# OpenRL-Lab/openrl

Measured on NVIDIA H100. Metric: env-steps/sec (collect+update), CartPole-v1 PPO, higher is better.
Workload: dtype f32 (nets, losses, Adam; the three 64x64 GEMM groups of the update run as split-fp16 wgmma MMAs with fp32 accumulation = fp32-class accuracy, the mode the 1e-4 parity tests run in), f64 (CartPole state)

## Files before the change

### openrl_b200/csrc/orl_fwd_tc.cu

```cuda
#include <algorithm>
#include <cstdlib>
#include <map>
#include <mutex>

#include "orl_envstep.cuh"
#include "orl_tc16.cuh"

namespace {
using namespace orl;
using namespace orl::tc;

constexpr int F_M = 128, F_NT = 256, FCW = 32;
constexpr uint32_t FPANEL = F_M * 16, FPANEL_W = H * 16;
constexpr int S_LD = 68;
constexpr uint32_t FOFF_R1H = 0, FOFF_R1L = 8 * FPANEL, FOFF_WH = 16 * FPANEL, FOFF_WL = FOFF_WH + 8 * FPANEL_W, FOFF_S = FOFF_WL + 8 * FPANEL_W,
                   FOFF_SMALL = FOFF_S + F_M * S_LD * 4;
constexpr uint32_t F_SMALL_FLOATS = 8 * H + H + H + MAX_OUT * H + MAX_OUT;
constexpr uint32_t F_XCH_FLOATS = 2 * F_M * 2 + 2 * F_M * 8 + F_M * 8;
constexpr uint32_t F_SMEM = FOFF_SMALL + 4 * (F_SMALL_FLOATS + F_XCH_FLOATS);

#define F_FOR_OUT(j) _Pragma("unroll") for (int j = 0; j < NOUT; ++j) if (NOUT != 8 || j < n)
#define F_ROWGROUP_SYNC()                                                      \
    do {                                                                       \
        switch (warp & 3) {                                                    \
// ... 76 lines not shown
    for (int i = 0; i < FCW; ++i) { n1[i] = f_act<ACT>(n1[i], activation_id); s += n1[i]; sq = fmaf(n1[i], n1[i], sq); }
    {
        *reinterpret_cast<float2*>(c.xs + (half * F_M + row) * 2) = make_float2(s, sq);
        F_ROWGROUP_SYNC();
        const float2 o = *reinterpret_cast<const float2*>(c.xs + ((half ^ 1) * F_M + row) * 2);
        s += o.x; sq += o.y;
    }
    const float mu1 = s * (1.f / H);
    const float rstd1 = 1.0f / sqrtf(fmaxf(sq * (1.f / H) - mu1 * mu1, 0.f) + LN_EPS);
#pragma unroll
    for (int i = 0; i < FCW; ++i) n1[i] = (n1[i] - mu1) * rstd1;
#pragma unroll
    for (int q8 = 0; q8 < FCW; q8 += 8) {
        const uint32_t off = (uint32_t)((cb + q8) >> 3) * FPANEL + row * 16;
        split_store8(c.R1h + off, c.R1l + off, n1 + q8, 1.0f);
    }
    fence_proxy_async();
    __syncthreads();
    {
        const uint64_t dK_A = desc_const(FPANEL, 128), dK_W = desc_const(FPANEL_W, 128);
        float z[32];
#pragma unroll
        for (int i = 0; i < 32; ++i) z[i] = 0.f;
        wgmma_fence();
#pragma unroll
        for (int pass = 0; pass < 3; ++pass) {
            const uint32_t aa = (pass == 0 ? c.aR1l : c.aR1h) + half * 64 * 16, bb = pass == 1 ? c.aWl : c.aWh;
#pragma unroll
            for (int kk = 0; kk < 4; ++kk)
                wgmma_f16_n64<0, 0>(z, desc_at(dK_A, aa + 2 * kk * FPANEL), desc_at(dK_W, bb + 2 * kk * FPANEL_W), (pass | kk) > 0);
        }
        wgmma_commit();
        overlap();
        wgmma_wait0();
        frag_store<64>(z, c.S + half * 64 * S_LD, S_LD);
    }
    __syncthreads();
    float n3[FCW];
#pragma unroll
    for (int q4 = 0; q4 < FCW; q4 += 4) {
        const float4 v = *reinterpret_cast<const float4*>(c.S + row * S_LD + cb + q4);
        n3[q4] = v.x; n3[q4 + 1] = v.y; n3[q4 + 2] = v.z; n3[q4 + 3] = v.w;
    }
    float s3 = 0.f, q3 = 0.f;
#pragma unroll
    for (int i = 0; i < FCW; ++i) { n3[i] += c.b3f[cb + i]; s3 += n3[i]; q3 = fmaf(n3[i], n3[i], q3); }
    {
        __syncwarp();
        *reinterpret_cast<float2*>(c.xs + (half * F_M + row) * 2) = make_float2(s3, q3);
        F_ROWGROUP_SYNC();
        const float2 o = *reinterpret_cast<const float2*>(c.xs + ((half ^ 1) * F_M + row) * 2);
        s3 += o.x; q3 += o.y;
    }
    const float mu3 = s3 * (1.f / H);
    const float rstd3 = 1.0f / sqrtf(fmaxf(q3 * (1.f / H) - mu3 * mu3, 0.f) + LN_EPS);
#pragma unroll
    for (int j = 0; j < MAX_OUT; ++j) out[j] = 0.f;
#pragma unroll
    for (int q4 = 0; q4 < FCW; q4 += 4) {
#pragma unroll
        for (int i = 0; i < 4; ++i) n3[q4 + i] = (n3[q4 + i] - mu3) * rstd3;
        F_FOR_OUT(j) {
            const float4 wv = *reinterpret_cast<const float4*>(c.whf + j * H + cb + q4);
            out[j] = fmaf(n3[q4], wv.x, fmaf(n3[q4 + 1], wv.y, fmaf(n3[q4 + 2], wv.z, fmaf(n3[q4 + 3], wv.w, out[j]))));
        }
    }
    {
// ... 229 lines not shown
            *reinterpret_cast<float2*>(xs + (qd * F_M + row) * 2) = make_float2(sm, sq);
            Q_ROWGROUP_SYNC();
            {
                sm = 0.f; sq = 0.f;
#pragma unroll
                for (int p = 0; p < 4; ++p) { const float2 o = *reinterpret_cast<const float2*>(xs + (p * F_M + row) * 2); sm += o.x; sq += o.y; }
            }
            const float mu1 = sm * (1.f / H);
            const float rstd1 = 1.0f / sqrtf(fmaxf(sq * (1.f / H) - mu1 * mu1, 0.f) + LN_EPS);
#pragma unroll
            for (int i = 0; i < QCW; ++i) n1[i] = (n1[i] - mu1) * rstd1;
#pragma unroll
            for (int q8 = 0; q8 < QCW; q8 += 8) {
                const uint32_t off = (uint32_t)((cb + q8) >> 3) * FPANEL + row * 16;
                split_store8(c.R1h + off, c.R1l + off, n1 + q8, 1.0f);
            }
            fence_proxy_async();
            Q_FWD_SYNC();
            {
                const uint64_t dK_A = desc_const(FPANEL, 128), dK_W = desc_const(FPANEL_W, 128);
                const int mb = qd & 1, nb = qd >> 1;
                float z[16];
#pragma unroll
                for (int i = 0; i < 16; ++i) z[i] = 0.f;
                wgmma_fence();
#pragma unroll
                for (int pass = 0; pass < 3; ++pass) {
                    const uint32_t aa = (pass == 0 ? c.aR1l : c.aR1h) + mb * 64 * 16, bb = (pass == 1 ? c.aWl : c.aWh) + nb * 32 * 16;
#pragma unroll
                    for (int kk = 0; kk < 4; ++kk)
                        wgmma_f16_n32<0, 0>(z, desc_at(dK_A, aa + 2 * kk * FPANEL), desc_at(dK_W, bb + 2 * kk * FPANEL_W), (pass | kk) > 0);
                }
                wgmma_commit();
                wgmma_wait0();
                frag_store<32>(z, c.S + mb * 64 * S_LD + 32 * nb, S_LD);
            }
            Q_FWD_SYNC();
            float n3[QCW];
#pragma unroll
            for (int q4 = 0; q4 < QCW; q4 += 4) {
                const float4 v = *reinterpret_cast<const float4*>(c.S + row * S_LD + cb + q4);
                n3[q4] = v.x; n3[q4 + 1] = v.y; n3[q4 + 2] = v.z; n3[q4 + 3] = v.w;
            }
            float s3 = 0.f, q3 = 0.f;
#pragma unroll
            for (int i = 0; i < QCW; ++i) { n3[i] += c.b3f[cb + i]; s3 += n3[i]; q3 = fmaf(n3[i], n3[i], q3); }
            __syncwarp();
            *reinterpret_cast<float2*>(xs + (qd * F_M + row) * 2) = make_float2(s3, q3);
            Q_ROWGROUP_SYNC();
            {
                s3 = 0.f; q3 = 0.f;
#pragma unroll
                for (int p = 0; p < 4; ++p) { const float2 o = *reinterpret_cast<const float2*>(xs + (p * F_M + row) * 2); s3 += o.x; q3 += o.y; }
            }
            const float mu3 = s3 * (1.f / H);
            const float rstd3 = 1.0f / sqrtf(fmaxf(q3 * (1.f / H) - mu3 * mu3, 0.f) + LN_EPS);
            float out[MAX_OUT];
#pragma unroll
            for (int j = 0; j < MAX_OUT; ++j) out[j] = 0.f;
#pragma unroll
            for (int q4 = 0; q4 < QCW; q4 += 4) {
#pragma unroll
                for (int i = 0; i < 4; ++i) n3[q4 + i] = (n3[q4 + i] - mu3) * rstd3;
                F_FOR_OUT(j) {
                    const float4 wv = *reinterpret_cast<const float4*>(c.whf + j * H + cb + q4);
                    out[j] = fmaf(n3[q4], wv.x, fmaf(n3[q4 + 1], wv.y, fmaf(n3[q4 + 2], wv.z, fmaf(n3[q4 + 3], wv.w, out[j]))));
                }
// ... 118 lines not shown
```

### openrl_b200/csrc/orl_ppo_tc.cu

```cuda
#include <cuda.h>

#include <algorithm>
#include <cstdlib>
#include <cstring>
#include <map>
#include <mutex>

#include "orl_mlp.cuh"
#include "orl_tc16.cuh"

namespace orl {
int ppo_stride_host(int obs_dim, int critic_obs_dim, int n_actions);
}

namespace {
using namespace orl;
using namespace orl::tc;

constexpr int T_M = 128, T_NT = 256;
constexpr int CW = 32;
constexpr uint32_t PANEL = T_M * 16;
constexpr uint32_t PANEL_W = H * 16;
constexpr int R1_PANELS = 10, R2_PANELS = 9;
constexpr int P_CST = 8, P_X = 9, P_U = 8;
constexpr int N_LOSS_TC = 8;
constexpr int S_LD = 68, GA_LD = 84, GB_LD = 20;
constexpr uint32_t OFF_R1H = 0, OFF_R1L = OFF_R1H + R1_PANELS * PANEL, OFF_R2H = OFF_R1L + R1_PANELS * PANEL,
                   OFF_R2L = OFF_R2H + R2_PANELS * PANEL, OFF_WH = OFF_R2L + R2_PANELS * PANEL, OFF_WL = OFF_WH + 8 * PANEL_W,
                   OFF_S = OFF_WL + 8 * PANEL_W, OFF_STAGE = OFF_S + T_M * S_LD * 4;
static_assert((T_M * GA_LD + 64 * GB_LD) * 4 <= OFF_WH, "the Ga / Gb staging fits in R1 + R2");
static_assert(OFF_STAGE % 128 == 0, "TMA destination alignment");
static_assert(OFF_R2L + 16 * PANEL <= OFF_STAGE + 4096, "the 16-panel A descriptors stay inside the allocation");
constexpr int N_SCAL = 4;

struct TcMaps {
    CUtensorMap obs_p, obs_c, actions, old_logp, adv, value_preds, returns, active;
};

struct AdvNormTc { float m0, s0, m1, s1; bool two; };

#define FOR_OUT(j) _Pragma("unroll") for (int j = 0; j < NOUT; ++j) if (NOUT != 8 || j < n)
#define ROWGROUP_SYNC()                                                        \
    do {                                                                       \
        switch (warp & 3) {                                                    \
            case 0: asm volatile("bar.sync 1, 64;" ::: "memory"); break;       \
            case 1: asm volatile("bar.sync 2, 64;" ::: "memory"); break;       \
            case 2: asm volatile("bar.sync 3, 64;" ::: "memory"); break;       \
            default: asm volatile("bar.sync 4, 64;" ::: "memory"); break;      \
        }                                                                      \
    } while (0)

__host__ __device__ inline uint32_t tc_stage_bytes(int d) { return (uint32_t)((T_M * d * 4 + 127) & ~127) + N_SCAL * T_M * 4; }
__host__ __device__ inline uint32_t tc_small_off(int d) { return OFF_STAGE + tc_stage_bytes(d); }
constexpr uint32_t SMALL_FLOATS = 8 * H + H + H + MAX_OUT * H + 2 * MAX_OUT;
constexpr uint32_t XCH_FLOATS = 2 * T_M * 2 + 2 * T_M * 8;
__host__ __device__ inline uint32_t tc_smem_bytes(int d) { return tc_small_off(d) + 4 * (SMALL_FLOATS + XCH_FLOATS) + 8; }

template <int ACT>
__device__ __forceinline__ float act_fwd_t(float z, int activation_id) { return ACT == 1 ? fmaxf(z, 0.f) : act_fwd(z, activation_id); }
template <int ACT>
__device__ __forceinline__ float act_bwd_t(float a, bool pos, int activation_id) { return ACT == 1 ? (pos ? 1.f : 0.f) : act_bwd(a, pos, activation_id); }

template <bool POLICY, int NOUT, int ACT, bool TMA>
__device__ __forceinline__ void tc_net_pass(const OrlPpoArgs& a, const TcMaps& maps, uint8_t* smem, int cta, int G, int stride) {
    const int d = POLICY ? a.obs_dim : a.critic_obs_dim;
    const int n = POLICY ? (NOUT == 8 ? a.n_actions : NOUT) : 1;
    const float* params = POLICY ? a.policy_params : a.critic_params;
    const float* obs = POLICY ? a.policy_obs : a.critic_obs;
    const int tid = threadIdx.x, warp = tid >> 5;
    const int row = tid & 127, half = tid >> 7;
    const int cb = CW * half;
    const NetOffsets po = net_offsets(d, n);

    uint8_t* R1h = smem + OFF_R1H; uint8_t* R1l = smem + OFF_R1L;
    uint8_t* R2h = smem + OFF_R2H; uint8_t* R2l = smem + OFF_R2L;
    uint8_t* Wh = smem + OFF_WH;   uint8_t* Wl = smem + OFF_WL;
    float* S = reinterpret_cast<float*>(smem + OFF_S);
    float* st_obs = reinterpret_cast<float*>(smem + OFF_STAGE);
    float* st_sc = reinterpret_cast<float*>(smem + OFF_STAGE + ((T_M * d * 4 + 127) & ~127));
    float* w1t = reinterpret_cast<float*>(smem + tc_small_off(d));
    float* b1s = w1t + 8 * H;
    float* b3f = b1s + H;
    float* whf = b3f + H;
    float* bhf = whf + MAX_OUT * H;
    float* swh = bhf + MAX_OUT;
    float* xs = swh + MAX_OUT;
    float* xh = xs + 2 * T_M * 2;
    uint64_t* bar_st = reinterpret_cast<uint64_t*>(xh + 2 * T_M * 8);

    for (int i = tid; i < 8 * H; i += T_NT) { const int k = i / H, j = i % H; w1t[i] = (k < d) ? params[po.w1 + j * d + k] : 0.f; }
    for (int i = tid; i < H; i += T_NT) b1s[i] = params[po.b1 + i];
    for (int i = tid; i < H * 8; i += T_NT) {
        const int pnl = i / H, j = i % H;
        float w8[8];
#pragma unroll
        for (int c = 0; c < 8; ++c) w8[c] = params[po.w3 + j * H + 8 * pnl + c] * params[po.g1 + 8 * pnl + c];
        const uint32_t off = (uint32_t)pnl * PANEL_W + j * 16;
        split_store8(Wh + off, Wl + off, w8, 1.0f);
    }
    for (int i = tid; i < MAX_OUT * H; i += T_NT) { const int j = i / H, k = i % H; whf[i] = (j < n) ? params[po.wh + j * H + k] * params[po.g3 + k] : 0.f; }
    for (int j = tid; j < H; j += T_NT) {
        float s = params[po.b3 + j];
        for (int k = 0; k < H; ++k) s = fmaf(params[po.w3 + j * H + k], params[po.be1 + k], s);
        b3f[j] = s;
    }
    for (int j = tid; j < MAX_OUT; j += T_NT) {
        float s = 0.f;
        if (j < n) { s = params[po.bh + j]; for (int k = 0; k < H; ++k) s = fmaf(params[po.wh + j * H + k], params[po.be3 + k], s); }
        bhf[j] = s;
        float rs = 0.f;
        if (j < n) for (int k = 0; k < H; ++k) rs += params[po.wh + j * H + k] * params[po.g3 + k];
        swh[j] = rs;
    }
    if (half == 0) {
        const uint4 z = make_uint4(0u, 0u, 0u, 0u);
        *reinterpret_cast<uint4*>(R1h + P_CST * PANEL + row * 16) = z; *reinterpret_cast<uint4*>(R1l + P_CST * PANEL + row * 16) = z;
        *reinterpret_cast<uint4*>(R1h + P_X * PANEL + row * 16) = z;   *reinterpret_cast<uint4*>(R1l + P_X * PANEL + row * 16) = z;
        *reinterpret_cast<uint4*>(R2h + P_U * PANEL + row * 16) = z;   *reinterpret_cast<uint4*>(R2l + P_U * PANEL + row * 16) = z;
    }
    if (tid == 0) mbar_init(bar_st, 1);
    fence_proxy_async();
// ... 14 lines not shown
    const int e_z = min(max(e_rows + 3 - (int)floorf(log2f(fmaxf(wmax, 1e-12f))), 0), 60);
    const float Sz = exp2f((float)e_z), Su = exp2f((float)e_u);
    constexpr float SX = 16.f, K1 = 0.25f;
    const float invSz = exp2f(-(float)e_z), invSu = exp2f(-(float)e_u), invS1 = invSz * (1.f / K1);
    AdvNormTc an = {0.f, 1.f, 0.f, 1.f, false};
    float vn_mean = 0.f, vn_std = 1.f;
    if (POLICY) {
        const double* gs = a.gae_stats;
        const double n_all = gs[ORL_GS_COUNT], n_act = gs[ORL_GS_ACT_COUNT];
        const double mean_all = gs[ORL_GS_ADV_SUM] / n_all;
        const double var_all = fmax(gs[ORL_GS_ADV_SQSUM] / n_all - mean_all * mean_all, 0.0);
        double mean_act = gs[ORL_GS_ADV_ACT_SUM] / n_act;
        double std_act = sqrt(fmax(gs[ORL_GS_ADV_ACT_SQSUM] / n_act - mean_act * mean_act, 0.0));
        if (a.flags & ORL_PPO_ADV_NORMALIZE) {
            const double s0 = (double)((float)sqrt(var_all)) + 1e-5;
            an.two = true; an.m0 = (float)mean_all; an.s0 = (float)s0;
            mean_act = (mean_act - mean_all) / s0; std_act = std_act / s0;
        }
        an.m1 = (float)mean_act; an.s1 = (float)((double)((float)std_act) + 1e-5);
    } else if (a.flags & ORL_PPO_VALUENORM) {
        const float bm = (float)(a.mb_stats[0] / rows_d), bsq = (float)(a.mb_stats[1] / rows_d);
        const float beta = (float)a.vn_beta, omw = (float)(1.0 - a.vn_beta);
        float st[3];
        st[0] = __fadd_rn(__fmul_rn(a.vn_state[0], beta), __fmul_rn(bm, omw));
        st[1] = __fadd_rn(__fmul_rn(a.vn_state[1], beta), __fmul_rn(bsq, omw));
        st[2] = __fadd_rn(__fmul_rn(a.vn_state[2], beta), __fmul_rn(1.0f, omw));
        const VnScalars s = vn_mean_std(st);
        vn_mean = s.mean; vn_std = s.std;
    }

    const uint64_t dK_A = desc_const(PANEL, 128), dK_W = desc_const(PANEL_W, 128);
    const uint64_t dMN_A = desc_const(128, PANEL), dMN_W = desc_const(128, PANEL_W);
    const uint32_t aR1h = smem_u32(R1h), aR1l = smem_u32(R1l), aR2h = smem_u32(R2h), aR2l = smem_u32(R2l), aWh = smem_u32(Wh), aWl = smem_u32(Wl);

    const long long n_tiles = (a.batch_rows + T_M - 1) / T_M;
    const float* sc0 = POLICY ? a.actions : a.value_preds;
    const float* sc1 = POLICY ? a.old_log_probs : a.returns;
    const float* sc2 = POLICY ? a.advantages : nullptr;
    const uint32_t stage_tx = (uint32_t)(T_M * d * 4) + (POLICY ? 4u : 3u) * T_M * 4;
    auto issue_tma = [&](long long tile) {
        const int r0 = (int)(a.row_begin + tile * T_M);
        mbar_expect_tx(bar_st, stage_tx);
        tma_load_2d(st_obs, POLICY ? &maps.obs_p : &maps.obs_c, 0, r0, bar_st);
        tma_load_1d(st_sc + 0 * T_M, POLICY ? &maps.actions : &maps.value_preds, r0, bar_st);
        tma_load_1d(st_sc + 1 * T_M, POLICY ? &maps.old_logp : &maps.returns, r0, bar_st);
        if (POLICY) tma_load_1d(st_sc + 2 * T_M, &maps.adv, r0, bar_st);
        tma_load_1d(st_sc + 3 * T_M, &maps.active, r0, bar_st);
    };
    auto issue_gather = [&](long long gi) {
        const bool v = gi >= 0;
        const long long g = v ? gi : 0;
        if (half == 0) {
            if ((d & 3) == 0) {
                for (int k = 0; k < d; k += 4) cp_async16(st_obs + row * d + k, obs + g * d + k, v);
            } else {
                for (int k = 0; k < d; ++k) cp_async4(st_obs + row * d + k, obs + g * d + k, v);
            }
        } else {
            cp_async4(st_sc + 0 * T_M + row, sc0 + g, v);
            cp_async4(st_sc + 1 * T_M + row, sc1 + g, v);
            if (POLICY) cp_async4(st_sc + 2 * T_M + row, sc2 + g, v);
            cp_async4(st_sc + 3 * T_M + row, a.active_masks + g, v);
        }
        cp_async_commit();
    };
    auto row_index = [&](long long tile) -> long long {
        if (tile >= n_tiles) return -1;
        const long long r = tile * T_M + row;
        if (r >= a.batch_rows) return -1;
        return a.indices ? a.indices[r] : a.row_begin + r;
    };
    long long gi_next = -1;
    if (TMA) {
        if (tid == 0 && cta < n_tiles) { tma_prefetch_desc(POLICY ? &maps.obs_p : &maps.obs_c); issue_tma(cta); }
    } else {
        issue_gather(row_index(cta));
        gi_next = row_index(cta + G);
    }
    long long gi = row_index(cta);

    float loss0 = 0.f, loss1 = 0.f, loss2 = 0.f;
    uint32_t it = 0;
    for (long long tile = cta; tile < n_tiles; tile += G, ++it) {
        const uint32_t par = it & 1u;
        if (TMA) mbar_wait(bar_st, par);
        else { cp_async_wait_all(); __syncthreads(); }
        const bool valid = gi >= 0;
        float x[8];
#pragma unroll
        for (int k = 0; k < 8; ++k) x[k] = 0.f;
        if (d == 4) {
            const float4 v = *reinterpret_cast<const float4*>(st_obs + row * 4);
            x[0] = v.x; x[1] = v.y; x[2] = v.z; x[3] = v.w;
        } else {
#pragma unroll
            for (int k = 0; k < 8; ++k) if (k < d) x[k] = st_obs[row * d + k];
        }
        const float row_a = st_sc[0 * T_M + row], row_b = st_sc[1 * T_M + row];
        const float row_c = POLICY ? st_sc[2 * T_M + row] : 0.f, active = st_sc[3 * T_M + row];

        float n1[CW];
#pragma unroll
        for (int q4 = 0; q4 < CW; q4 += 4) {
            const float4 b = *reinterpret_cast<const float4*>(b1s + cb + q4);
            n1[q4] = b.x; n1[q4 + 1] = b.y; n1[q4 + 2] = b.z; n1[q4 + 3] = b.w;
        }
#pragma unroll
        for (int k = 0; k < 8; ++k) {
            if (k < d) {
#pragma unroll
                for (int q4 = 0; q4 < CW; q4 += 4) {
                    const float4 wv = *reinterpret_cast<const float4*>(w1t + k * H + cb + q4);
                    n1[q4] = fmaf(x[k], wv.x, n1[q4]); n1[q4 + 1] = fmaf(x[k], wv.y, n1[q4 + 1]);
                    n1[q4 + 2] = fmaf(x[k], wv.z, n1[q4 + 2]); n1[q4 + 3] = fmaf(x[k], wv.w, n1[q4 + 3]);
                }
            }
        }
        unsigned posmask = 0u;
        float s = 0.f, sq = 0.f;
#pragma unroll
        for (int i = 0; i < CW; ++i) {
            if (n1[i] > 0.f) posmask |= 1u << i;
            n1[i] = act_fwd_t<ACT>(n1[i], a.activation_id);
            s += n1[i]; sq = fmaf(n1[i], n1[i], sq);
        }
        {
            *reinterpret_cast<float2*>(xs + (half * T_M + row) * 2) = make_float2(s, sq);
            ROWGROUP_SYNC();
            const float2 o = *reinterpret_cast<const float2*>(xs + ((half ^ 1) * T_M + row) * 2);
            s += o.x; sq += o.y;
        }
        const float mu1 = s * (1.f / H);
        const float rstd1 = 1.0f / sqrtf(fmaxf(sq * (1.f / H) - mu1 * mu1, 0.f) + LN_EPS);
#pragma unroll
        for (int i = 0; i < CW; ++i) n1[i] = (n1[i] - mu1) * rstd1;

        if (it > 0) __syncthreads();
#pragma unroll
        for (int q8 = 0; q8 < CW; q8 += 8) {
            const uint32_t off = (uint32_t)((cb + q8) >> 3) * PANEL + row * 16;
            split_store8(R1h + off, R1l + off, n1 + q8, 1.0f);
        }
        if (half == 0) split_store8(R1h + P_X * PANEL + row * 16, R1l + P_X * PANEL + row * 16, x, SX);
        fence_proxy_async();
        __syncthreads();
        float z[32];
#pragma unroll
        for (int i = 0; i < 32; ++i) z[i] = 0.f;
        wgmma_fence();
#pragma unroll
        for (int pass = 0; pass < 3; ++pass) {
            const uint32_t aa = (pass == 0 ? aR1l : aR1h) + half * 64 * 16, bb = pass == 1 ? aWl : aWh;
#pragma unroll
            for (int kk = 0; kk < 4; ++kk)
                wgmma_f16_n64<0, 0>(z, desc_at(dK_A, aa + 2 * kk * PANEL), desc_at(dK_W, bb + 2 * kk * PANEL_W), (pass | kk) > 0);
        }
        wgmma_commit();
        if (TMA && tid == 0 && tile + G < n_tiles) issue_tma(tile + G);
        long long gi_cur = gi;
        if (!TMA) {
            issue_gather(gi_next);
            gi = gi_next;
            gi_next = row_index(tile + 2 * G);
        } else {
            gi = row_index(tile + G);
        }

        wgmma_wait0();
        frag_store<64>(z, S + half * 64 * S_LD, S_LD);
        __syncthreads();

        float n3[CW];
#pragma unroll
        for (int q4 = 0; q4 < CW; q4 += 4) {
            const float4 v = *reinterpret_cast<const float4*>(S + row * S_LD + cb + q4);
            n3[q4] = v.x; n3[q4 + 1] = v.y; n3[q4 + 2] = v.z; n3[q4 + 3] = v.w;
        }
        float s3 = 0.f, q3 = 0.f;
#pragma unroll
        for (int i = 0; i < CW; ++i) { n3[i] += b3f[cb + i]; s3 += n3[i]; q3 = fmaf(n3[i], n3[i], q3); }
        {
            *reinterpret_cast<float2*>(xs + (half * T_M + row) * 2) = make_float2(s3, q3);
            ROWGROUP_SYNC();
            const float2 o = *reinterpret_cast<const float2*>(xs + ((half ^ 1) * T_M + row) * 2);
            s3 += o.x; q3 += o.y;
        }
        const float mu3 = s3 * (1.f / H);
        const float var3 = fmaxf(q3 * (1.f / H) - mu3 * mu3, 0.f) + LN_EPS;
        const float rstd3 = 1.0f / sqrtf(var3);
        float out[MAX_OUT];
#pragma unroll
        for (int j = 0; j < MAX_OUT; ++j) out[j] = 0.f;
#pragma unroll
        for (int q4 = 0; q4 < CW; q4 += 4) {
#pragma unroll
            for (int i = 0; i < 4; ++i) n3[q4 + i] = (n3[q4 + i] - mu3) * rstd3;
            FOR_OUT(j) {
                const float4 wv = *reinterpret_cast<const float4*>(whf + j * H + cb + q4);
                out[j] = fmaf(n3[q4], wv.x, fmaf(n3[q4 + 1], wv.y, fmaf(n3[q4 + 2], wv.z, fmaf(n3[q4 + 3], wv.w, out[j]))));
            }
        }
        {
            FOR_OUT(j) xh[(j * 2 + half) * T_M + row] = out[j];
            ROWGROUP_SYNC();
            FOR_OUT(j) out[j] += xh[(j * 2 + (half ^ 1)) * T_M + row];
        }
        float dot[MAX_OUT];
#pragma unroll
        for (int j = 0; j < MAX_OUT; ++j) { dot[j] = out[j]; out[j] += (j < NOUT && j < n) ? bhf[j] : 0.f; }

        float dl[MAX_OUT];
#pragma unroll
        for (int j = 0; j < MAX_OUT; ++j) dl[j] = 0.f;
        if (valid) {
            if (POLICY) {
                unsigned masked = 0;
                if (a.action_masks) {
#pragma unroll
                    for (int j = 0; j < MAX_OUT; ++j)
                        if (j < n && a.action_masks[gi_cur * n + j] == 0.f) { out[j] = -6e4f; masked |= 1u << j; }
                }
                float nl[MAX_OUT], pr[MAX_OUT];
                log_softmax_n(out, n, nl, pr);
                const int act = (int)row_a;
                float lp = nl[0];
#pragma unroll
                for (int j = 1; j < MAX_OUT; ++j) if (j == act) lp = nl[j];
                float adv = row_c;
                if (an.two) adv = (adv - an.m0) / an.s0;
                adv = (adv - an.m1) / an.s1;
                const PgTerm pg = pg_term(lp, row_b, adv, a.clip_param, a.flags, a.dual_clip_coeff);
                const float wrow = pol_masks ? active * inv_act : inv_rows;
                float ent = 0.f;
#pragma unroll
                for (int j = 0; j < MAX_OUT; ++j) if (j < n) ent -= pr[j] * nl[j];
                if (half == 0) { loss0 += pg.loss * wrow; loss1 += ent * wrow; loss2 += pg.ratio; }
                const float dlp = pg.dlogp * wrow, went = a.entropy_coef * wrow;
#pragma unroll
                for (int j = 0; j < MAX_OUT; ++j)
// ... 22 lines not shown
        }
        float m1 = 0.f, m2 = 0.f;
#pragma unroll
        for (int j = 0; j < MAX_OUT; ++j) dl[j] *= Sz;
        FOR_OUT(j) { m1 = fmaf(dl[j], swh[j], m1); m2 = fmaf(dl[j], dot[j], m2); }
        m1 *= (1.f / H); m2 *= (1.f / H);
#pragma unroll
        for (int q8 = 0; q8 < CW; q8 += 8) {
            float g8[8];
#pragma unroll
            for (int i = 0; i < 8; ++i) g8[i] = 0.f;
#pragma unroll
            for (int q4 = 0; q4 < 8; q4 += 4) {
                FOR_OUT(j) {
                    const float4 wv = *reinterpret_cast<const float4*>(whf + j * H + cb + q8 + q4);
                    g8[q4] = fmaf(dl[j], wv.x, g8[q4]); g8[q4 + 1] = fmaf(dl[j], wv.y, g8[q4 + 1]);
                    g8[q4 + 2] = fmaf(dl[j], wv.z, g8[q4 + 2]); g8[q4 + 3] = fmaf(dl[j], wv.w, g8[q4 + 3]);
                }
            }
#pragma unroll
            for (int i = 0; i < 8; ++i) g8[i] = rstd3 * (g8[i] - m1 - n3[q8 + i] * m2);
            const uint32_t off = (uint32_t)((cb + q8) >> 3) * PANEL + row * 16;
            split_store8(R2h + off, R2l + off, g8, 1.0f);
        }
        if (half == 0) {
            float u8[8], c8[8];
#pragma unroll
            for (int j = 0; j < 8; ++j) { u8[j] = dl[j] * (rstd3 * (Su * invSz)); c8[j] = 0.f; }
            c8[0] = 1.0f; c8[1] = mu3; c8[2] = var3 * rstd3;
            split_store8(R2h + P_U * PANEL + row * 16, R2l + P_U * PANEL + row * 16, u8, 1.0f);
            split_store8(R1h + P_CST * PANEL + row * 16, R1l + P_CST * PANEL + row * 16, c8, 1.0f);
        }
        fence_proxy_async();
        __syncthreads();
#pragma unroll
        for (int i = 0; i < 32; ++i) z[i] = 0.f;
        wgmma_fence();
#pragma unroll
        for (int pass = 0; pass < 3; ++pass) {
            const uint32_t aa = (pass == 0 ? aR2l : aR2h) + half * 64 * 16, bb = pass == 1 ? aWl : aWh;
#pragma unroll
            for (int kk = 0; kk < 4; ++kk)
                wgmma_f16_n64<0, 1>(z, desc_at(dK_A, aa + 2 * kk * PANEL), desc_at(dMN_W, bb + kk * 256), (pass | kk) > 0);
        }
#pragma unroll
        for (int pass = 0; pass < 3; ++pass) {
            const uint32_t aa = (pass == 0 ? aR2l : aR2h) + half * 8 * PANEL, bb = pass == 1 ? aR1l : aR1h;
#pragma unroll
            for (int kk = 0; kk < 8; ++kk)
                wgmma_f16_n80<1, 1>(ga, desc_at(dMN_A, aa + kk * 256), desc_at(dMN_A, bb + kk * 256), 1u);
        }
        wgmma_commit();
        wgmma_wait0();
        frag_store<64>(z, S + half * 64 * S_LD, S_LD);
        __syncthreads();
        {
            float g[CW];
#pragma unroll
            for (int q4 = 0; q4 < CW; q4 += 4) {
                const float4 v = *reinterpret_cast<const float4*>(S + row * S_LD + cb + q4);
                g[q4] = v.x; g[q4 + 1] = v.y; g[q4 + 2] = v.z; g[q4 + 3] = v.w;
            }
            float t1 = 0.f, t2 = 0.f;
#pragma unroll
            for (int i = 0; i < CW; ++i) { t1 += g[i]; t2 = fmaf(g[i], n1[i], t2); }
            {
                *reinterpret_cast<float2*>(xs + (half * T_M + row) * 2) = make_float2(t1, t2);
                ROWGROUP_SYNC();
                const float2 o = *reinterpret_cast<const float2*>(xs + ((half ^ 1) * T_M + row) * 2);
                t1 += o.x; t2 += o.y;
            }
            t1 *= (1.f / H); t2 *= (1.f / H);
            const float std1 = 1.0f / rstd1;
#pragma unroll
            for (int i = 0; i < CW; ++i) {
                const float da = rstd1 * (g[i] - t1 - n1[i] * t2);
                const float aval = fmaf(n1[i], std1, mu1);
                g[i] = da * (K1 * act_bwd_t<ACT>(aval, (posmask >> i) & 1u, a.activation_id));
            }
#pragma unroll
            for (int q8 = 0; q8 < CW; q8 += 8) {
                const uint32_t off = (uint32_t)((cb + q8) >> 3) * PANEL + row * 16;
                split_store8(R1h + off, R1l + off, g + q8, 1.0f);
            }
        }
        fence_proxy_async();
        __syncthreads();
        if (half == 1) {
            wgmma_fence();
#pragma unroll
            for (int pass = 0; pass < 3; ++pass) {
                const uint32_t aa = pass == 0 ? aR1l : aR1h, bb = (pass == 1 ? aR1l : aR1h) + P_CST * PANEL;
#pragma unroll
                for (int kk = 0; kk < 8; ++kk)
                    wgmma_f16_n16<1, 1>(gb, desc_at(dMN_A, aa + kk * 256), desc_at(dMN_A, bb + kk * 256), 1u);
            }
            wgmma_commit();
            wgmma_wait0();
        }
    }

    float* part = a.partials + (size_t)((POLICY ? 0 : G) + cta) * stride;
    const FoldOffsets fo = fold_offsets(d, n);
    float* qs = xh;
    float* qsu = qs + MAX_OUT * H;
    if (it > 0) {
        float* gas = reinterpret_cast<float*>(smem);
        float* gbs = gas + T_M * GA_LD;
        __syncthreads();
        frag_store<80>(ga, gas + half * 64 * GA_LD, GA_LD);
        if (half == 1) frag_store<16>(gb, gbs, GB_LD);
        __syncthreads();
        {
            float v[32];
#pragma unroll
            for (int c = 0; c < 32; ++c) v[c] = gas[row * GA_LD + 32 * half + c];
            if (row < H) {
#pragma unroll
                for (int c = 0; c < 32; ++c) part[fo.g3 + row * H + 32 * half + c] = v[c] * invSz;
            } else if (row < H + n) {
#pragma unroll
                for (int c = 0; c < 32; ++c) qs[(row - H) * H + 32 * half + c] = v[c];
            }
        }
        if (half == 0) {
            const float* c8 = gas + row * GA_LD + 64;
            if (row < H) part[fo.db3 + row] = c8[0] * invSz;
            else if (row < H + n) { qsu[row - H] = c8[0]; qsu[8 + row - H] = c8[1]; qsu[16 + row - H] = c8[2]; }
            if (row < H) {
                const float* g16 = gbs + row * GB_LD;
                part[fo.db1 + row] = g16[0] * invS1;
#pragma unroll
                for (int c = 0; c < 8; ++c) if (c < d) part[fo.g1 + row * d + c] = g16[8 + c] * (invS1 * (1.f / SX));
            }
        }
        __syncthreads();
        for (int o = tid; o < n * H; o += T_NT) {
            const int j = o >> 6, k = o & 63;
            float acc = 0.f;
            for (int i = 0; i < H; ++i) acc = fmaf(qs[j * H + i], params[po.w3 + k * H + i] * params[po.g1 + i], acc);
            acc = fmaf(b3f[k], qsu[j], acc) - qsu[8 + j];
            part[fo.gh + o] = acc * invSu;
            if (k == 0) { part[fo.dbh + j] = qsu[16 + j] * invSu; part[fo.dls + j] = 0.f; }
        }
    } else {
        for (int i = tid; i < fo.total; i += T_NT) part[i] = 0.f;
    }
    {
        float v[3] = {loss0, loss1, loss2};
        float* red = xs;
        const int lane = tid & 31;
        __syncthreads();
#pragma unroll
        for (int k = 0; k < 3; ++k) { const float sv = warp_sum(v[k]); if (lane == 0) red[k * 8 + warp] = sv; }
        __syncthreads();
        if (tid < N_LOSS_TC) {
            float sv = 0.f;
            if (tid < 3) for (int wv = 0; wv < T_NT / 32; ++wv) sv += red[tid * 8 + wv];
            part[stride - N_LOSS_TC + tid] = sv;
        }
    }
}

template <int NOUT, int ACT, bool TMA>
__global__ void __launch_bounds__(T_NT, 1) ppo_fwdbwd_tc_kernel(const OrlPpoArgs a, const __grid_constant__ TcMaps maps, int stride) {
    extern __shared__ __align__(1024) uint8_t smem_tc[];
    const int G = a.grid_per_net;
    const bool policy = (int)blockIdx.x < G;
    const int cta = policy ? (int)blockIdx.x : (int)blockIdx.x - G;
    if (policy) tc_net_pass<true, NOUT, ACT, TMA>(a, maps, smem_tc, cta, G, stride);
    else tc_net_pass<false, 1, ACT, TMA>(a, maps, smem_tc, cta, G, stride);
}

using TcKernel = void (*)(const OrlPpoArgs, const TcMaps, int);
template <int NOUT, int ACT>
TcKernel pick_staging(bool tma) { return tma ? ppo_fwdbwd_tc_kernel<NOUT, ACT, true> : ppo_fwdbwd_tc_kernel<NOUT, ACT, false>; }
template <int NOUT>
TcKernel pick_act(int activation_id, bool tma) { return activation_id == 1 ? pick_staging<NOUT, 1>(tma) : pick_staging<NOUT, -1>(tma); }
TcKernel pick_kernel(int n_actions, int activation_id, bool tma) {
    if (n_actions == 2) return pick_act<2>(activation_id, tma);
    if (n_actions == 5) return pick_act<5>(activation_id, tma);
    return pick_act<8>(activation_id, tma);
}

// ... 94 lines not shown
```

### openrl_b200/csrc/orl_tc.cuh

```cuda
#pragma once
#include <cuda_runtime.h>
#include <stdint.h>

namespace orl {
namespace tc {

__device__ __forceinline__ uint32_t smem_u32(const void* p) { return (uint32_t)__cvta_generic_to_shared(p); }

__device__ __forceinline__ void fence_proxy_async() { asm volatile("fence.proxy.async.shared::cta;" ::: "memory"); }

__device__ __forceinline__ void mbar_init(uint64_t* bar, uint32_t count) {
    asm volatile("mbarrier.init.shared::cta.b64 [%0], %1;" ::"r"(smem_u32(bar)), "r"(count) : "memory");
    asm volatile("fence.mbarrier_init.release.cluster;" ::: "memory");
}
__device__ __forceinline__ void mbar_wait(uint64_t* bar, uint32_t parity) {
    const uint32_t a = smem_u32(bar);
    asm volatile(
        "{\n\t.reg .pred p;\n\t"
        "WAIT_LOOP:\n\t"
        "mbarrier.try_wait.parity.shared::cta.b64 p, [%0], %1;\n\t"
        "@p bra DONE;\n\t"
        "bra WAIT_LOOP;\n\t"
        "DONE:\n\t}" ::"r"(a), "r"(parity) : "memory");
}

__device__ __forceinline__ void wgmma_fence() { asm volatile("wgmma.fence.sync.aligned;" ::: "memory"); }
__device__ __forceinline__ void wgmma_commit() { asm volatile("wgmma.commit_group.sync.aligned;" ::: "memory"); }
__device__ __forceinline__ void wgmma_wait0() { asm volatile("wgmma.wait_group.sync.aligned 0;" ::: "memory"); }

template <int TA, int TB>
__device__ __forceinline__ void wgmma_f16_n16(float (&d)[8], uint64_t desc_a, uint64_t desc_b, uint32_t accumulate) {
    asm volatile(
        "{\n\t.reg .pred p;\n\t"
        "setp.ne.b32 p, %10, 0;\n\t"
        "wgmma.mma_async.sync.aligned.m64n16k16.f32.f16.f16 "
        "{%0,%1,%2,%3,%4,%5,%6,%7}, %8, %9, p, 1, 1, %11, %12;\n\t}"
        : "+f"(d[0]), "+f"(d[1]), "+f"(d[2]), "+f"(d[3]), "+f"(d[4]), "+f"(d[5]), "+f"(d[6]), "+f"(d[7])
        : "l"(desc_a), "l"(desc_b), "r"(accumulate), "n"(TA), "n"(TB)
        : "memory");
}
template <int TA, int TB>
__device__ __forceinline__ void wgmma_f16_n32(float (&d)[16], uint64_t desc_a, uint64_t desc_b, uint32_t accumulate) {
    asm volatile(
        "{\n\t.reg .pred p;\n\t"
        "setp.ne.b32 p, %18, 0;\n\t"
        "wgmma.mma_async.sync.aligned.m64n32k16.f32.f16.f16 "
        "{%0,%1,%2,%3,%4,%5,%6,%7,%8,%9,%10,%11,%12,%13,%14,%15}, %16, %17, p, 1, 1, %19, %20;\n\t}"
        : "+f"(d[0]), "+f"(d[1]), "+f"(d[2]), "+f"(d[3]), "+f"(d[4]), "+f"(d[5]), "+f"(d[6]), "+f"(d[7]), "+f"(d[8]), "+f"(d[9]), "+f"(d[10]), "+f"(d[11]), "+f"(d[12]), "+f"(d[13]), "+f"(d[14]), "+f"(d[15])
        : "l"(desc_a), "l"(desc_b), "r"(accumulate), "n"(TA), "n"(TB)
        : "memory");
}
template <int TA, int TB>
__device__ __forceinline__ void wgmma_f16_n64(float (&d)[32], uint64_t desc_a, uint64_t desc_b, uint32_t accumulate) {
    asm volatile(
        "{\n\t.reg .pred p;\n\t"
        "setp.ne.b32 p, %34, 0;\n\t"
        "wgmma.mma_async.sync.aligned.m64n64k16.f32.f16.f16 "
        "{%0,%1,%2,%3,%4,%5,%6,%7,%8,%9,%10,%11,%12,%13,%14,%15,%16,%17,%18,%19,%20,%21,%22,%23,%24,%25,%26,%27,%28,%29,%30,%31}, %32, %33, p, 1, 1, %35, %36;\n\t}"
        : "+f"(d[0]), "+f"(d[1]), "+f"(d[2]), "+f"(d[3]), "+f"(d[4]), "+f"(d[5]), "+f"(d[6]), "+f"(d[7]), "+f"(d[8]), "+f"(d[9]), "+f"(d[10]), "+f"(d[11]), "+f"(d[12]), "+f"(d[13]), "+f"(d[14]), "+f"(d[15]), "+f"(d[16]), "+f"(d[17]), "+f"(d[18]), "+f"(d[19]), "+f"(d[20]), "+f"(d[21]), "+f"(d[22]), "+f"(d[23]), "+f"(d[24]), "+f"(d[25]), "+f"(d[26]), "+f"(d[27]), "+f"(d[28]), "+f"(d[29]), "+f"(d[30]), "+f"(d[31])
        : "l"(desc_a), "l"(desc_b), "r"(accumulate), "n"(TA), "n"(TB)
        : "memory");
// ... 26 lines not shown
```

Before: 202.7 million.

## Remap PPO update rows per warpgroup, use shuffles and split barriers

Changes the PPO update kernel's thread-to-row mapping so each row's two column halves live in the same warp. The cross-half LayerNorm and head reductions can then use warp shuffles instead of shared-memory exchanges plus named barriers. Most CTA-wide __syncthreads are replaced by per-warpgroup named barriers or __syncwarp. A new R3 smem region lets the gradient-B GEMM run asynchronously across iterations, using bar.arrive/bar.sync and wgmma_wait<N> to keep the Ga GEMM in flight while the S fragment is consumed. This costs extra shared memory and adds subtle ordering risk around buffer reuse.

```diff
diff --git a/openrl_b200/csrc/orl_fwd_tc.cu b/openrl_b200/csrc/orl_fwd_tc.cu
--- a/openrl_b200/csrc/orl_fwd_tc.cu
+++ b/openrl_b200/csrc/orl_fwd_tc.cu
@@ -132,7 +132,7 @@
         }
         wgmma_commit();
         overlap();
-        wgmma_wait0();
+        wgmma_wait<0>();
         frag_store<64>(z, c.S + half * 64 * S_LD, S_LD);
     }
     __syncthreads();
@@ -428,7 +428,7 @@
                         wgmma_f16_n32<0, 0>(z, desc_at(dK_A, aa + 2 * kk * FPANEL), desc_at(dK_W, bb + 2 * kk * FPANEL_W), (pass | kk) > 0);
                 }
                 wgmma_commit();
-                wgmma_wait0();
+                wgmma_wait<0>();
                 frag_store<32>(z, c.S + mb * 64 * S_LD + 32 * nb, S_LD);
             }
             Q_FWD_SYNC();
diff --git a/openrl_b200/csrc/orl_ppo_tc.cu b/openrl_b200/csrc/orl_ppo_tc.cu
--- a/openrl_b200/csrc/orl_ppo_tc.cu
+++ b/openrl_b200/csrc/orl_ppo_tc.cu
@@ -21,16 +21,17 @@
 constexpr int CW = 32;
 constexpr uint32_t PANEL = T_M * 16;
 constexpr uint32_t PANEL_W = H * 16;
-constexpr int R1_PANELS = 10, R2_PANELS = 9;
+constexpr int R1_PANELS = 10, R2_PANELS = 9, R3_PANELS = 8;
 constexpr int P_CST = 8, P_X = 9, P_U = 8;
 constexpr int N_LOSS_TC = 8;
 constexpr int S_LD = 68, GA_LD = 84, GB_LD = 20;
 constexpr uint32_t OFF_R1H = 0, OFF_R1L = OFF_R1H + R1_PANELS * PANEL, OFF_R2H = OFF_R1L + R1_PANELS * PANEL,
                    OFF_R2L = OFF_R2H + R2_PANELS * PANEL, OFF_WH = OFF_R2L + R2_PANELS * PANEL, OFF_WL = OFF_WH + 8 * PANEL_W,
-                   OFF_S = OFF_WL + 8 * PANEL_W, OFF_STAGE = OFF_S + T_M * S_LD * 4;
+                   OFF_R3H = OFF_WL + 8 * PANEL_W, OFF_R3L = OFF_R3H + R3_PANELS * PANEL,
+                   OFF_S = OFF_R3L + R3_PANELS * PANEL, OFF_STAGE = OFF_S + T_M * S_LD * 4;
 static_assert((T_M * GA_LD + 64 * GB_LD) * 4 <= OFF_WH, "the Ga / Gb staging fits in R1 + R2");
 static_assert(OFF_STAGE % 128 == 0, "TMA destination alignment");
-static_assert(OFF_R2L + 16 * PANEL <= OFF_STAGE + 4096, "the 16-panel A descriptors stay inside the allocation");
+static_assert(OFF_R2L + 16 * PANEL <= OFF_R3H, "the 16-panel A descriptors of GEMM3a stop short of R3 (written while they run)");
 constexpr int N_SCAL = 4;
 
 struct TcMaps {
@@ -40,20 +41,13 @@
 struct AdvNormTc { float m0, s0, m1, s1; bool two; };
 
 #define FOR_OUT(j) _Pragma("unroll") for (int j = 0; j < NOUT; ++j) if (NOUT != 8 || j < n)
-#define ROWGROUP_SYNC()                                                        \
-    do {                                                                       \
-        switch (warp & 3) {                                                    \
-            case 0: asm volatile("bar.sync 1, 64;" ::: "memory"); break;       \
-            case 1: asm volatile("bar.sync 2, 64;" ::: "memory"); break;       \
-            case 2: asm volatile("bar.sync 3, 64;" ::: "memory"); break;       \
-            default: asm volatile("bar.sync 4, 64;" ::: "memory"); break;      \
-        }                                                                      \
-    } while (0)
+__device__ __forceinline__ float other_half(float v) { return __shfl_xor_sync(0xffffffffu, v, 16); }
+__device__ __forceinline__ void warpgroup_sync(int g) { asm volatile("bar.sync %0, 128;" ::"r"(1 + g) : "memory"); }
 
 __host__ __device__ inline uint32_t tc_stage_bytes(int d) { return (uint32_t)((T_M * d * 4 + 127) & ~127) + N_SCAL * T_M * 4; }
 __host__ __device__ inline uint32_t tc_small_off(int d) { return OFF_STAGE + tc_stage_bytes(d); }
 constexpr uint32_t SMALL_FLOATS = 8 * H + H + H + MAX_OUT * H + 2 * MAX_OUT;
-constexpr uint32_t XCH_FLOATS = 2 * T_M * 2 + 2 * T_M * 8;
+constexpr uint32_t XCH_FLOATS = MAX_OUT * H + 3 * MAX_OUT + 3 * 8;
 __host__ __device__ inline uint32_t tc_smem_bytes(int d) { return tc_small_off(d) + 4 * (SMALL_FLOATS + XCH_FLOATS) + 8; }
 
 template <int ACT>
@@ -67,14 +61,15 @@
     const int n = POLICY ? (NOUT == 8 ? a.n_actions : NOUT) : 1;
     const float* params = POLICY ? a.policy_params : a.critic_params;
     const float* obs = POLICY ? a.policy_obs : a.critic_obs;
-    const int tid = threadIdx.x, warp = tid >> 5;
-    const int row = tid & 127, half = tid >> 7;
+    const int tid = threadIdx.x, warp = tid >> 5, lane = tid & 31;
+    const int row = 16 * warp + (lane & 15), half = lane >> 4, wg = warp >> 2;
     const int cb = CW * half;
     const NetOffsets po = net_offsets(d, n);
 
     uint8_t* R1h = smem + OFF_R1H; uint8_t* R1l = smem + OFF_R1L;
     uint8_t* R2h = smem + OFF_R2H; uint8_t* R2l = smem + OFF_R2L;
     uint8_t* Wh = smem + OFF_WH;   uint8_t* Wl = smem + OFF_WL;
+    uint8_t* R3h = smem + OFF_R3H; uint8_t* R3l = smem + OFF_R3L;
     float* S = reinterpret_cast<float*>(smem + OFF_S);
     float* st_obs = reinterpret_cast<float*>(smem + OFF_STAGE);
     float* st_sc = reinterpret_cast<float*>(smem + OFF_STAGE + ((T_M * d * 4 + 127) & ~127));
@@ -84,9 +79,9 @@
     float* whf = b3f + H;
     float* bhf = whf + MAX_OUT * H;
     float* swh = bhf + MAX_OUT;
-    float* xs = swh + MAX_OUT;
-    float* xh = xs + 2 * T_M * 2;
-    uint64_t* bar_st = reinterpret_cast<uint64_t*>(xh + 2 * T_M * 8);
+    float* qs = swh + MAX_OUT;
+    float* red = qs + MAX_OUT * H + 3 * MAX_OUT;
+    uint64_t* bar_st = reinterpret_cast<uint64_t*>(red + 3 * 8);
 
     for (int i = tid; i < 8 * H; i += T_NT) { const int k = i / H, j = i % H; w1t[i] = (k < d) ? params[po.w1 + j * d + k] : 0.f; }
     for (int i = tid; i < H; i += T_NT) b1s[i] = params[po.b1 + i];
@@ -167,6 +162,7 @@
     const uint64_t dK_A = desc_const(PANEL, 128), dK_W = desc_const(PANEL_W, 128);
     const uint64_t dMN_A = desc_const(128, PANEL), dMN_W = desc_const(128, PANEL_W);
     const uint32_t aR1h = smem_u32(R1h), aR1l = smem_u32(R1l), aR2h = smem_u32(R2h), aR2l = smem_u32(R2l), aWh = smem_u32(Wh), aWl = smem_u32(Wl);
+    const uint32_t aR3h = smem_u32(R3h), aR3l = smem_u32(R3l);
 
     const long long n_tiles = (a.batch_rows + T_M - 1) / T_M;
     const float* sc0 = POLICY ? a.actions : a.value_preds;
@@ -219,7 +215,7 @@
     for (long long tile = cta; tile < n_tiles; tile += G, ++it) {
         const uint32_t par = it & 1u;
         if (TMA) mbar_wait(bar_st, par);
-        else { cp_async_wait_all(); __syncthreads(); }
+        else { cp_async_wait_all(); __syncwarp(); }
         const bool valid = gi >= 0;
         float x[8];
 #pragma unroll
@@ -259,18 +255,14 @@
             n1[i] = act_fwd_t<ACT>(n1[i], a.activation_id);
             s += n1[i]; sq = fmaf(n1[i], n1[i], sq);
         }
-        {
-            *reinterpret_cast<float2*>(xs + (half * T_M + row) * 2) = make_float2(s, sq);
-            ROWGROUP_SYNC();
-            const float2 o = *reinterpret_cast<const float2*>(xs + ((half ^ 1) * T_M + row) * 2);
-            s += o.x; sq += o.y;
-        }
+        wgmma_wait<0>();
+        s += other_half(s); sq += other_half(sq);
         const float mu1 = s * (1.f / H);
         const float rstd1 = 1.0f / sqrtf(fmaxf(sq * (1.f / H) - mu1 * mu1, 0.f) + LN_EPS);
 #pragma unroll
         for (int i = 0; i < CW; ++i) n1[i] = (n1[i] - mu1) * rstd1;
 
-        if (it > 0) __syncthreads();
+        __syncthreads();
 #pragma unroll
         for (int q8 = 0; q8 < CW; q8 += 8) {
             const uint32_t off = (uint32_t)((cb + q8) >> 3) * PANEL + row * 16;
@@ -278,14 +270,14 @@
         }
         if (half == 0) split_store8(R1h + P_X * PANEL + row * 16, R1l + P_X * PANEL + row * 16, x, SX);
         fence_proxy_async();
-        __syncthreads();
+        warpgroup_sync(wg);
         float z[32];
 #pragma unroll
         for (int i = 0; i < 32; ++i) z[i] = 0.f;
         wgmma_fence();
 #pragma unroll
         for (int pass = 0; pass < 3; ++pass) {
-            const uint32_t aa = (pass == 0 ? aR1l : aR1h) + half * 64 * 16, bb = pass == 1 ? aWl : aWh;
+            const uint32_t aa = (pass == 0 ? aR1l : aR1h) + wg * 64 * 16, bb = pass == 1 ? aWl : aWh;
 #pragma unroll
             for (int kk = 0; kk < 4; ++kk)
                 wgmma_f16_n64<0, 0>(z, desc_at(dK_A, aa + 2 * kk * PANEL), desc_at(dK_W, bb + 2 * kk * PANEL_W), (pass | kk) > 0);
@@ -301,9 +293,9 @@
             gi = row_index(tile + G);
         }
 
-        wgmma_wait0();
-        frag_store<64>(z, S + half * 64 * S_LD, S_LD);
-        __syncthreads();
+        wgmma_wait<0>();
+        frag_store<64>(z, S + wg * 64 * S_LD, S_LD);
+        __syncwarp();
 
         float n3[CW];
 #pragma unroll
@@ -314,12 +306,7 @@
         float s3 = 0.f, q3 = 0.f;
 #pragma unroll
         for (int i = 0; i < CW; ++i) { n3[i] += b3f[cb + i]; s3 += n3[i]; q3 = fmaf(n3[i], n3[i], q3); }
-        {
-            *reinterpret_cast<float2*>(xs + (half * T_M + row) * 2) = make_float2(s3, q3);
-            ROWGROUP_SYNC();
-            const float2 o = *reinterpret_cast<const float2*>(xs + ((half ^ 1) * T_M + row) * 2);
-            s3 += o.x; q3 += o.y;
-        }
+        s3 += other_half(s3); q3 += other_half(q3);
         const float mu3 = s3 * (1.f / H);
         const float var3 = fmaxf(q3 * (1.f / H) - mu3 * mu3, 0.f) + LN_EPS;
         const float rstd3 = 1.0f / sqrtf(var3);
@@ -335,11 +322,7 @@
                 out[j] = fmaf(n3[q4], wv.x, fmaf(n3[q4 + 1], wv.y, fmaf(n3[q4 + 2], wv.z, fmaf(n3[q4 + 3], wv.w, out[j]))));
             }
         }
-        {
-            FOR_OUT(j) xh[(j * 2 + half) * T_M + row] = out[j];
-            ROWGROUP_SYNC();
-            FOR_OUT(j) out[j] += xh[(j * 2 + (half ^ 1)) * T_M + row];
-        }
+        FOR_OUT(j) out[j] += other_half(out[j]);
         float dot[MAX_OUT];
 #pragma unroll
         for (int j = 0; j < MAX_OUT; ++j) { dot[j] = out[j]; out[j] += (j < NOUT && j < n) ? bhf[j] : 0.f; }
@@ -428,28 +411,30 @@
             split_store8(R1h + P_CST * PANEL + row * 16, R1l + P_CST * PANEL + row * 16, c8, 1.0f);
         }
         fence_proxy_async();
-        __syncthreads();
+        warpgroup_sync(wg);
 #pragma unroll
         for (int i = 0; i < 32; ++i) z[i] = 0.f;
         wgmma_fence();
 #pragma unroll
         for (int pass = 0; pass < 3; ++pass) {
-            const uint32_t aa = (pass == 0 ? aR2l : aR2h) + half * 64 * 16, bb = pass == 1 ? aWl : aWh;
+            const uint32_t aa = (pass == 0 ? aR2l : aR2h) + wg * 64 * 16, bb = pass == 1 ? aWl : aWh;
 #pragma unroll
             for (int kk = 0; kk < 4; ++kk)
                 wgmma_f16_n64<0, 1>(z, desc_at(dK_A, aa + 2 * kk * PANEL), desc_at(dMN_W, bb + kk * 256), (pass | kk) > 0);
         }
+        wgmma_commit();
+        __syncthreads();
 #pragma unroll
         for (int pass = 0; pass < 3; ++pass) {
-            const uint32_t aa = (pass == 0 ? aR2l : aR2h) + half * 8 * PANEL, bb = pass == 1 ? aR1l : aR1h;
+            const uint32_t aa = (pass == 0 ? aR2l : aR2h) + wg * 8 * PANEL, bb = pass == 1 ? aR1l : aR1h;
 #pragma unroll
             for (int kk = 0; kk < 8; ++kk)
                 wgmma_f16_n80<1, 1>(ga, desc_at(dMN_A, aa + kk * 256), desc_at(dMN_A, bb + kk * 256), 1u);
         }
         wgmma_commit();
-        wgmma_wait0();
-        frag_store<64>(z, S + half * 64 * S_LD, S_LD);
-        __syncthreads();
+        wgmma_wait<1>();
+        frag_store<64>(z, S + wg * 64 * S_LD, S_LD);
+        __syncwarp();
         {
             float g[CW];
 #pragma unroll
@@ -460,12 +445,7 @@
             float t1 = 0.f, t2 = 0.f;
 #pragma unroll
             for (int i = 0; i < CW; ++i) { t1 += g[i]; t2 = fmaf(g[i], n1[i], t2); }
-            {
-                *reinterpret_cast<float2*>(xs + (half * T_M + row) * 2) = make_float2(t1, t2);
-                ROWGROUP_SYNC();
-                const float2 o = *reinterpret_cast<const float2*>(xs + ((half ^ 1) * T_M + row) * 2);
-                t1 += o.x; t2 += o.y;
-            }
+            t1 += other_half(t1); t2 += other_half(t2);
             t1 *= (1.f / H); t2 *= (1.f / H);
             const float std1 = 1.0f / rstd1;
 #pragma unroll
@@ -477,35 +457,36 @@
 #pragma unroll
             for (int q8 = 0; q8 < CW; q8 += 8) {
                 const uint32_t off = (uint32_t)((cb + q8) >> 3) * PANEL + row * 16;
-                split_store8(R1h + off, R1l + off, g + q8, 1.0f);
+                split_store8(R3h + off, R3l + off, g + q8, 1.0f);
             }
         }
         fence_proxy_async();
-        __syncthreads();
-        if (half == 1) {
+        if (wg == 1) {
+            asm volatile("bar.sync 3, 256;" ::: "memory");
             wgmma_fence();
 #pragma unroll
             for (int pass = 0; pass < 3; ++pass) {
-                const uint32_t aa = pass == 0 ? aR1l : aR1h, bb = (pass == 1 ? aR1l : aR1h) + P_CST * PANEL;
+                const uint32_t aa = pass == 0 ? aR3l : aR3h, bb = (pass == 1 ? aR1l : aR1h) + P_CST * PANEL;
 #pragma unroll
                 for (int kk = 0; kk < 8; ++kk)
                     wgmma_f16_n16<1, 1>(gb, desc_at(dMN_A, aa + kk * 256), desc_at(dMN_A, bb + kk * 256), 1u);
             }
             wgmma_commit();
-            wgmma_wait0();
-        }
-    }
+        } else {
+            asm volatile("bar.arrive 3, 256;" ::: "memory");
+        }
+    }
+    wgmma_wait<0>();
 
     float* part = a.partials + (size_t)((POLICY ? 0 : G) + cta) * stride;
     const FoldOffsets fo = fold_offsets(d, n);
-    float* qs = xh;
     float* qsu = qs + MAX_OUT * H;
     if (it > 0) {
         float* gas = reinterpret_cast<float*>(smem);
         float* gbs = gas + T_M * GA_LD;
         __syncthreads();
-        frag_store<80>(ga, gas + half * 64 * GA_LD, GA_LD);
-        if (half == 1) frag_store<16>(gb, gbs, GB_LD);
+        frag_store<80>(ga, gas + wg * 64 * GA_LD, GA_LD);
+        if (wg == 1) frag_store<16>(gb, gbs, GB_LD);
         __syncthreads();
         {
             float v[32];
@@ -544,8 +525,6 @@
     }
     {
         float v[3] = {loss0, loss1, loss2};
-        float* red = xs;
-        const int lane = tid & 31;
         __syncthreads();
 #pragma unroll
         for (int k = 0; k < 3; ++k) { const float sv = warp_sum(v[k]); if (lane == 0) red[k * 8 + warp] = sv; }
diff --git a/openrl_b200/csrc/orl_tc.cuh b/openrl_b200/csrc/orl_tc.cuh
--- a/openrl_b200/csrc/orl_tc.cuh
+++ b/openrl_b200/csrc/orl_tc.cuh
@@ -26,7 +26,8 @@
 
 __device__ __forceinline__ void wgmma_fence() { asm volatile("wgmma.fence.sync.aligned;" ::: "memory"); }
 __device__ __forceinline__ void wgmma_commit() { asm volatile("wgmma.commit_group.sync.aligned;" ::: "memory"); }
-__device__ __forceinline__ void wgmma_wait0() { asm volatile("wgmma.wait_group.sync.aligned 0;" ::: "memory"); }
+template <int N>
+__device__ __forceinline__ void wgmma_wait() { asm volatile("wgmma.wait_group.sync.aligned %0;" ::"n"(N) : "memory"); }
 
 template <int TA, int TB>
 __device__ __forceinline__ void wgmma_f16_n16(float (&d)[8], uint64_t desc_a, uint64_t desc_b, uint32_t accumulate) {
```

New measurement: 212.4 million (median of 6 runs). 1.05x the previous value.
